# ghnmqdtg/VM-ASR

Measured on AMD Instinct MI355X. Metric: audio clips/sec (train step) 48kHz n_fft=1024, higher is better.
Workload: dtype bf16 (autocast over G; scan/STFT f32; MPD f32/bf16x3 MFMA); 1 GPU; vm_asr_48k_MPD.yaml full train step, DIMS 16 d_state 1 n_fft 1024 clip 122640@48k; per_gpu_batch=4, global_batch=4, parallelism=dp1, execution=hipGraph replay, 2 streams, generator_streams=2

## Files before the change

include/vmasr_hip.h:

```cpp
#ifndef VMASR_HIP_H
#define VMASR_HIP_H

#include <stddef.h>
#include <stdint.h>

#ifdef __cplusplus
extern "C" {
#endif

#define VMASR_ABI_VERSION 1

typedef void *vmasr_stream_t;

enum { VMASR_F32 = 0, VMASR_F16 = 1, VMASR_BF16 = 2 };

enum {
    VMASR_OK = 0,
    VMASR_EINVAL = -1,
    VMASR_EALIGN = -2,
    VMASR_ENOSPACE = -3
};

int vmasr_abi_version(void);
const char *vmasr_last_error(void);
// ... 36 lines not shown
void vmasr_sscan_tune(int rows, int split);

int vmasr_cross_scan(const void *x, void *xs, int32_t B, int32_t C, int32_t H, int32_t W,
                     int32_t dtype, vmasr_stream_t stream);
int vmasr_cross_merge(const void *ys, void *y, int32_t B, int32_t C, int32_t H, int32_t W,
                      int32_t dtype, vmasr_stream_t stream);

int vmasr_cross_scan_cvt(const void *x, void *xs, int32_t B, int32_t C, int32_t H, int32_t W,
                         int32_t in_dtype, int32_t out_dtype, vmasr_stream_t stream);
int vmasr_cross_merge_cvt(const void *ys, void *y, int32_t B, int32_t C, int32_t H, int32_t W,
                          int32_t in_dtype, int32_t out_dtype, vmasr_stream_t stream);

int vmasr_xproj_n_supported(int32_t d_state, int32_t dt_rank, int32_t d_inner);
size_t vmasr_xproj_n_ws_floats(int32_t B, int32_t K, int32_t R, int32_t L);
int vmasr_xproj_n_fwd(const void *xs, const float *Wx, const float *Wdt, float *dts, float *Bs, float *Cs, float *dtr,
                      int32_t B, int32_t K, int32_t D, int32_t N, int32_t R, int32_t L, int32_t dtype, vmasr_stream_t stream);
int vmasr_xproj_n_bwd(const void *xs, const float *Wx, const float *Wdt, const float *dtr, const float *ddts, const float *dBs,
                      const float *dCs, const float *du, void *dxs, float *dWx, float *dWdt, float *ws,
                      int32_t B, int32_t K, int32_t D, int32_t N, int32_t R, int32_t L, int32_t dtype, vmasr_stream_t stream);
int vmasr_xproj_supported(int32_t d_state, int32_t dt_rank, int32_t d_inner);
int vmasr_xproj_fwd(const void *xs, const float *Wx, const float *Wdt, float *dts, float *Bs, float *Cs,
                    float *dtr, int32_t B, int32_t K, int32_t D, int32_t N, int32_t R, int32_t L,
                    int32_t dtype, vmasr_stream_t stream);
int vmasr_xproj_bwd(const void *xs, const float *Wx, const float *Wdt, const float *dtr, const float *ddts,
                    const float *dBs, const float *dCs, const float *du, void *dxs, float *dWx, float *dWdt,
                    float *ws, int32_t B, int32_t K, int32_t D, int32_t N, int32_t R, int32_t L,
                    int32_t dtype, vmasr_stream_t stream);

int vmasr_dwconv_silu_fwd(const void *x, const float *w, const float *bias, void *y, int32_t B,
                          int32_t C, int32_t H, int32_t W, int32_t dtype, vmasr_stream_t stream);
int vmasr_dwconv_silu_bwd(const void *x, const float *w, const float *bias, const void *gy,
                          void *dx, float *dw, float *db, float *ws, int32_t B, int32_t C,
                          int32_t H, int32_t W, int32_t dtype, vmasr_stream_t stream);

int vmasr_stft(const float *wav, float *out0, float *out1, int32_t B, int32_t T, int32_t n_fft,
               int32_t hop, int32_t win, int32_t normalized, int32_t logmag,
               vmasr_stream_t stream);
size_t vmasr_stft_bwd_workspace(int32_t B, int32_t T, int32_t n_fft, int32_t hop);
int vmasr_stft_bwd(const float *gre, const float *gim, float *gwav, int32_t B, int32_t T, int32_t n_fft,
                   int32_t hop, int32_t win, int32_t normalized, void *ws, size_t ws_bytes,
                   vmasr_stream_t stream);
size_t vmasr_istft_workspace(int32_t B, int32_t F, int32_t M, int32_t hop);
int vmasr_istft(const float *mag, const float *phase, float *wav, int32_t B, int32_t F, int32_t M,
                int32_t hop, int32_t win, void *ws, size_t ws_bytes, vmasr_stream_t stream);
int vmasr_istft_bwd(const float *mag, const float *phase, const float *g, float *dmag,
                    float *dphase, int32_t B, int32_t F, int32_t M, int32_t hop, int32_t win,
                    vmasr_stream_t stream);

enum { VMASR_SCALE_LOG2 = 0, VMASR_SCALE_DB = 1 };
size_t vmasr_stft_db_workspace(int32_t B, int32_t T, int32_t n_fft, int32_t hop);
int vmasr_stft_db(const float *wav, float *mag, float *phase, int32_t B, int32_t T, int32_t n_fft, int32_t hop,
                  int32_t win, int32_t normalized, float top_db, void *ws, size_t ws_bytes, vmasr_stream_t stream);
int vmasr_istft_scaled(const float *mag, const float *phase, float *wav, int32_t B, int32_t F, int32_t M, int32_t hop,
                       int32_t win, int32_t scale, void *ws, size_t ws_bytes, vmasr_stream_t stream);
int vmasr_istft_scaled_bwd(const float *mag, const float *phase, const float *g, float *dmag, float *dphase, int32_t B,
                           int32_t F, int32_t M, int32_t hop, int32_t win, int32_t scale, vmasr_stream_t stream);

size_t vmasr_metrics_workspace(int32_t B, int32_t T, int32_t n_fft, int32_t hop);
int vmasr_metrics(const float *out, const float *tgt, const int64_t *hf, float *per_clip, double *acc, int32_t B, int32_t T,
                  int32_t n_fft, int32_t hop, void *ws, size_t ws_bytes, vmasr_stream_t stream);

int vmasr_resample_poly(const float *x, const float *h, float *y, int32_t B, int64_t n_in, int64_t n_out, int32_t up, int32_t down,
                        int32_t half_len, vmasr_stream_t stream);

size_t vmasr_resample_design_workspace(int32_t half_len);
int vmasr_resample_design(float *h, int32_t up, int32_t down, int32_t half_len, void *ws, size_t ws_bytes, vmasr_stream_t stream);
// ... 289 lines not shown

int32_t vmasr_dconv1d_pos_tile(void);
int32_t vmasr_dconv1d_m_tile(void);
int32_t vmasr_dconv1d_k_chunk(void);
int32_t vmasr_dconv1d_max_taps(void);
int vmasr_dconv1d_supported(int32_t Cin, int32_t Cout, int32_t groups, int32_t k, int32_t stride);
int vmasr_dconv1d_supported_launch(int32_t Cin, int32_t Cout, int32_t groups, int32_t k, int32_t stride, int32_t pad, int32_t B, int64_t L);
int32_t vmasr_dconv1d_fwd_slabs(int32_t Cin, int32_t Cout, int32_t groups, int32_t k, int32_t stride, int32_t pad, int32_t B, int64_t L);
size_t vmasr_dconv1d_fwd_workspace(int32_t Cin, int32_t Cout, int32_t groups, int32_t k, int32_t stride, int32_t pad, int32_t B, int64_t L);
size_t vmasr_dconv1d_dgrad_workspace(int32_t Cin, int32_t Cout, int32_t groups, int32_t k, int32_t stride, int32_t pad, int32_t B, int64_t L);
size_t vmasr_dconv1d_wgrad_workspace(int32_t Cin, int32_t Cout, int32_t groups, int32_t k, int32_t stride, int32_t pad, int32_t B, int64_t L);
int vmasr_dconv1d_fwd(const float *x, const float *w, const float *bias, float *y, float *pre, void *ws, size_t ws_bytes, int32_t B,
                      int32_t Cin, int32_t Cout, int32_t groups, int64_t L, int32_t k, int32_t stride, int32_t pad, int32_t act,
                      vmasr_stream_t stream);
int vmasr_dconv1d_dgrad(const float *gy, const float *pre, const float *w, float *dx, void *ws, size_t ws_bytes, int32_t B, int32_t Cin,
                        int32_t Cout, int32_t groups, int64_t L, int32_t k, int32_t stride, int32_t pad, vmasr_stream_t stream);
int vmasr_dconv1d_wgrad(const float *x, const float *gy, const float *pre, float *dw, float *db, void *ws, size_t ws_bytes, int32_t B,
                        int32_t Cin, int32_t Cout, int32_t groups, int64_t L, int32_t k, int32_t stride, int32_t pad, vmasr_stream_t stream);

enum {
    VMASR_K_SSCAN_FWD = 0,
    VMASR_K_SSCAN_FWD_AGG,
    VMASR_K_SSCAN_FWD_CARRY,
    VMASR_K_SSCAN_FWD_APPLY,
    VMASR_K_SSCAN_BWD,
    VMASR_K_SSCAN_BWD_AGG,
    VMASR_K_SSCAN_BWD_CARRY,
    VMASR_K_SSCAN_BWD_APPLY,
    VMASR_K_CROSS_SCAN,
    VMASR_K_CROSS_MERGE,
    VMASR_K_DWCONV_FWD,
    VMASR_K_DWCONV_BWD_A,
    VMASR_K_DWCONV_BWD_B,
    VMASR_K_STFT,
    VMASR_K_ISTFT_FRAMES,
    VMASR_K_ISTFT_OLA,
    VMASR_K_ISTFT_BWD,
    VMASR_K_LN_FWD,
    VMASR_K_LN_BWD,
    VMASR_K_LN_BWD_REDUCE,
    VMASR_K_SMALL_LINEAR_FWD,
    VMASR_K_SMALL_LINEAR_BWD,
    VMASR_K_SMALL_LINEAR_REDUCE,
    VMASR_K_XPROJ_FWD,
    VMASR_K_XPROJ_BWD_A,
    VMASR_K_XPROJ_BWD_B,
    VMASR_K_SPECTRAL,
    VMASR_K_IM2COL,
    VMASR_K_COL2IM,
    VMASR_K_SPLIT_BF16,
    VMASR_K_BIAS_GELU,
    VMASR_K_SS2D_TRANSPOSE,
    VMASR_K_SS2D_FWD_AGG,
    VMASR_K_SS2D_CARRY,
    VMASR_K_SS2D_FWD_APPLY,
    VMASR_K_SS2D_MERGE,
    VMASR_K_SS2D_BWD_AGG,
    VMASR_K_SS2D_BWD_APPLY,
    VMASR_K_SS2D_PRE,
    VMASR_K_LN_GATE,
    VMASR_K_STACK_ROWS,
    VMASR_K_FEAT_L1,
    VMASR_K_ADAMW,
    VMASR_K_CONV_POST,
    VMASR_K_CONV_POST_BWD_GELU,
    VMASR_K_WEIGHT_T,
// ... 59 lines not shown
```

vm_asr_amd/_lib.py:

```python
import ctypes
import os

from . import knobs

_HERE = os.path.dirname(os.path.abspath(__file__))
LIB_PATH = knobs.get("VMASR_LIB") or os.path.join(_HERE, "libvmasr_hip.so")

c_i32, c_i64, c_vp, c_sz = ctypes.c_int32, ctypes.c_int64, ctypes.c_void_p, ctypes.c_size_t

F32, F16, BF16 = 0, 1, 2


class SScanParams(ctypes.Structure):
    _fields_ = (
        [(n, c_i32) for n in ("batch", "dim", "seqlen", "dstate", "n_groups", "n_chunks", "dtype",
                              "delta_softplus")]
        + [(n, c_i64) for n in ("A_d_stride", "A_dstate_stride",
                                "B_batch_stride", "B_group_stride", "B_dstate_stride",
                                "C_batch_stride", "C_group_stride", "C_dstate_stride",
                                "u_batch_stride", "u_d_stride", "delta_batch_stride", "delta_d_stride",
                                "out_batch_stride", "out_d_stride")]
        + [(n, c_vp) for n in ("A_ptr", "B_ptr", "C_ptr", "D_ptr", "u_ptr", "delta_ptr",
                               "delta_bias_ptr", "out_ptr", "x_ptr")]
    )
# ... 135 lines not shown
    "vmasr_ss2d_glue_supported": (ctypes.c_int, [c_i32, c_i32, c_i32]),
    "vmasr_ss2d_pre_fwd": (ctypes.c_int, [c_vp, c_vp, c_vp, c_i32, c_i32, c_i32, c_i32, c_vp]),
    "vmasr_ss2d_pre_bwd": (ctypes.c_int, [c_vp, c_vp, c_vp, c_vp, c_i32, c_i32, c_i32, c_i32, c_vp]),
    "vmasr_ln_gate_fwd": (ctypes.c_int, [c_vp] * 7 + [c_i32, c_i32, c_i32, ctypes.c_float, c_i32, c_vp]),
    "vmasr_ln_gate_bwd": (ctypes.c_int, [c_vp] * 11 + [c_i32, c_i32, c_i32, c_i32, c_vp]),
    "vmasr_ln_gate_bwd_workspace": (c_i64, [c_i32, c_i32, c_i32, c_i32]),
    "vmasr_ln_gate_bwd_ws": (ctypes.c_int, [c_vp] * 12 + [c_i32, c_i32, c_i32, c_i32, c_vp]),
    "vmasr_ln_gate_pair_supported": (ctypes.c_int, [c_i32, c_i32, c_i32]),
    "vmasr_ln_gate_pair_fwd": (ctypes.c_int, [c_vp] * 8 + [c_i32, c_i32, c_i32, c_i32, ctypes.c_float, c_i32, c_vp]),
    "vmasr_ln_gate_pair_bwd": (ctypes.c_int, [c_vp] * 13 + [c_i32, c_i32, c_i32, c_i32, c_i32, c_vp]),
    "vmasr_ss2d_supported": (ctypes.c_int, [c_i32] * 5),
    "vmasr_ss2d_part_floats": (c_sz, [c_i32] * 4),
    "vmasr_ss2d_fwd": (ctypes.c_int, [ctypes.POINTER(SS2DParams), c_vp]),
    "vmasr_ss2d_bwd": (ctypes.c_int, [ctypes.POINTER(SS2DParams), c_vp]),
    "vmasr_ss2d_deep_supported": (ctypes.c_int, [c_i32] * 5),
    "vmasr_ss2d_deep_waves_per_row": (c_i32, [c_i32, c_i32]),
    "vmasr_ss2d_deep_fwd": (ctypes.c_int, [ctypes.POINTER(SS2DDeepParams), c_vp]),
    "vmasr_ss2d_deep_bwd": (ctypes.c_int, [ctypes.POINTER(SS2DDeepParams), c_vp]),
    "vmasr_set_deterministic": (None, [ctypes.c_int]),
    "vmasr_get_deterministic": (ctypes.c_int, []),
    "vmasr_det_timeouts": (ctypes.c_int64, []),
    "vmasr_prof_enable": (None, [ctypes.c_int]),
    "vmasr_prof_reset": (None, []),
    "vmasr_prof_name": (ctypes.c_char_p, [ctypes.c_int]),
    "vmasr_prof_collect": (ctypes.c_int, [ctypes.c_int, ctypes.POINTER(ctypes.c_int64),
                                          ctypes.POINTER(ctypes.c_double), ctypes.POINTER(ctypes.c_double)]),
    "vmasr_prof_collect_shapes": (ctypes.c_int, [ctypes.c_int, ctypes.c_int, ctypes.POINTER(ctypes.c_double), ctypes.POINTER(ctypes.c_int64),
                                                 ctypes.POINTER(ctypes.c_double)]),
    "vmasr_cross_scan": (ctypes.c_int, [c_vp, c_vp, c_i32, c_i32, c_i32, c_i32, c_i32, c_vp]),
    "vmasr_cross_merge": (ctypes.c_int, [c_vp, c_vp, c_i32, c_i32, c_i32, c_i32, c_i32, c_vp]),
    "vmasr_dwconv_silu_fwd": (ctypes.c_int, [c_vp, c_vp, c_vp, c_vp, c_i32, c_i32, c_i32, c_i32, c_i32, c_vp]),
    "vmasr_dwconv_silu_bwd": (ctypes.c_int, [c_vp, c_vp, c_vp, c_vp, c_vp, c_vp, c_vp, c_vp,
                                             c_i32, c_i32, c_i32, c_i32, c_i32, c_vp]),
    "vmasr_stft": (ctypes.c_int, [c_vp, c_vp, c_vp, c_i32, c_i32, c_i32, c_i32, c_i32, c_i32, c_i32, c_vp]),
    "vmasr_stft_bwd_workspace": (c_sz, [c_i32, c_i32, c_i32, c_i32]),
    "vmasr_stft_bwd": (ctypes.c_int, [c_vp, c_vp, c_vp, c_i32, c_i32, c_i32, c_i32, c_i32, c_i32, c_vp, c_sz, c_vp]),
    "vmasr_istft_workspace": (c_sz, [c_i32, c_i32, c_i32, c_i32]),
    "vmasr_istft": (ctypes.c_int, [c_vp, c_vp, c_vp, c_i32, c_i32, c_i32, c_i32, c_i32, c_vp, c_sz, c_vp]),
    "vmasr_istft_bwd": (ctypes.c_int, [c_vp, c_vp, c_vp, c_vp, c_vp, c_i32, c_i32, c_i32, c_i32, c_i32, c_vp]),
    "vmasr_stft_db_workspace": (c_sz, [c_i32, c_i32, c_i32, c_i32]),
    "vmasr_stft_db": (ctypes.c_int, [c_vp, c_vp, c_vp, c_i32, c_i32, c_i32, c_i32, c_i32, c_i32, ctypes.c_float, c_vp, c_sz, c_vp]),
    "vmasr_istft_scaled": (ctypes.c_int, [c_vp, c_vp, c_vp, c_i32, c_i32, c_i32, c_i32, c_i32, c_i32, c_vp, c_sz, c_vp]),
    "vmasr_istft_scaled_bwd": (ctypes.c_int, [c_vp, c_vp, c_vp, c_vp, c_vp, c_i32, c_i32, c_i32, c_i32, c_i32, c_i32, c_vp]),
    "vmasr_metrics_workspace": (c_sz, [c_i32, c_i32, c_i32, c_i32]),
    "vmasr_metrics": (ctypes.c_int, [c_vp, c_vp, c_vp, c_vp, c_vp, c_i32, c_i32, c_i32, c_i32, c_vp, c_sz, c_vp]),
    "vmasr_gconv1d_supported": (ctypes.c_int, [c_i32] * 5),
    "vmasr_gconv1d_supported_launch": (ctypes.c_int, [c_i32] * 7 + [c_i64]),
    "vmasr_gconv1d_wgrad_workspace": (c_sz, [c_i32] * 7 + [c_i64]),
    "vmasr_gconv1d_fwd": (ctypes.c_int, [c_vp] * 5 + [c_i32] * 4 + [c_i64] + [c_i32] * 4 + [c_vp]),
    "vmasr_gconv1d_dgrad": (ctypes.c_int, [c_vp] * 4 + [c_i32] * 4 + [c_i64] + [c_i32] * 3 + [c_vp]),
    "vmasr_gconv1d_wgrad": (ctypes.c_int, [c_vp] * 6 + [c_sz] + [c_i32] * 4 + [c_i64] + [c_i32] * 3 + [c_vp]),
    "vmasr_dconv1d_pos_tile": (c_i32, []),
    "vmasr_dconv1d_m_tile": (c_i32, []),
    "vmasr_dconv1d_k_chunk": (c_i32, []),
    "vmasr_dconv1d_max_taps": (c_i32, []),
    "vmasr_dconv1d_supported": (ctypes.c_int, [c_i32] * 5),
    "vmasr_dconv1d_supported_launch": (ctypes.c_int, [c_i32] * 7 + [c_i64]),
    "vmasr_dconv1d_fwd_slabs": (c_i32, [c_i32] * 7 + [c_i64]),
    "vmasr_dconv1d_fwd_workspace": (c_sz, [c_i32] * 7 + [c_i64]),
    "vmasr_dconv1d_dgrad_workspace": (c_sz, [c_i32] * 7 + [c_i64]),
    "vmasr_dconv1d_wgrad_workspace": (c_sz, [c_i32] * 7 + [c_i64]),
    "vmasr_dconv1d_fwd": (ctypes.c_int, [c_vp] * 6 + [c_sz] + [c_i32] * 4 + [c_i64] + [c_i32] * 4 + [c_vp]),
    "vmasr_dconv1d_dgrad": (ctypes.c_int, [c_vp] * 5 + [c_sz] + [c_i32] * 4 + [c_i64] + [c_i32] * 3 + [c_vp]),
    "vmasr_dconv1d_wgrad": (ctypes.c_int, [c_vp] * 6 + [c_sz] + [c_i32] * 4 + [c_i64] + [c_i32] * 3 + [c_vp]),
    "vmasr_stem1d_time_tile": (c_i32, []),
    "vmasr_stem1d_channel_group": (c_i32, []),
# ... 2 lines not shown
    "vmasr_stem1d_bwd_workspace": (c_sz, [c_i32] * 5 + [c_i64]),
    "vmasr_stem1d_fwd": (ctypes.c_int, [c_vp] * 4 + [c_i32] * 2 + [c_i64] + [c_i32] * 4 + [c_vp]),
    "vmasr_stem1d_bwd": (ctypes.c_int, [c_vp] * 8 + [c_sz] + [c_i32] * 2 + [c_i64] + [c_i32] * 4 + [c_vp]),
    "vmasr_stem1d_fm_supported_launch": (ctypes.c_int, [c_i32] * 5 + [c_i64]),
    "vmasr_stem1d_fm_workspace": (c_sz, [c_i32] * 5 + [c_i64]),
    "vmasr_stem1d_fm_fwd": (ctypes.c_int, [c_vp] * 6 + [c_sz] + [c_i32] * 2 + [c_i64] + [c_i32] * 3 + [c_vp]),
    "vmasr_stem1d_fm_bwd": (ctypes.c_int, [c_vp] * 6 + [ctypes.c_float] + [c_vp] + [c_i32] * 2 + [c_i64] + [c_i32] * 3 + [c_vp]),
    "vmasr_resample_poly": (ctypes.c_int, [c_vp, c_vp, c_vp, c_i32, c_i64, c_i64, c_i32, c_i32, c_i32, c_vp]),
    "vmasr_resample_design_workspace": (c_sz, [c_i32]),
    "vmasr_resample_design": (ctypes.c_int, [c_vp, c_i32, c_i32, c_i32, c_vp, c_sz, c_vp]),
    "vmasr_degrade_batch_workspace": (c_sz, [c_vp, c_i32]),
    "vmasr_degrade_batch": (ctypes.c_int, [c_vp, c_vp, c_vp, c_vp, c_i32, c_i64, c_vp, c_sz, c_vp]),
}

_lib = None


def lib():
    global _lib
    if _lib is None:
        if not os.path.exists(LIB_PATH):
            raise RuntimeError(
                f"{LIB_PATH} is missing: build it with `make -C vm_asr_amd/csrc` "
                "(or __graft_entry__.build()). vm_asr_amd has no CPU fallback.")
        import torch
        l = ctypes.CDLL(LIB_PATH)
        for name, (res, args) in SYMBOLS.items():
            fn = getattr(l, name)
            fn.restype, fn.argtypes = res, args
        if l.vmasr_abi_version() != 1:
            raise RuntimeError("libvmasr_hip.so ABI version mismatch")
        if knobs.get("VMASR_DETERMINISTIC"):
            l.vmasr_set_deterministic(1)
        knobs.warn_undeclared()
        _lib = l
    return _lib


def check(code, what):
    if code != 0:
        msg = lib().vmasr_last_error().decode() or "unknown error"
        raise RuntimeError(f"{what} failed ({code}): {msg}")


def torch_dtype_code(dt):
    import torch
    try:
        return {torch.float32: F32, torch.float16: F16, torch.bfloat16: BF16}[dt]
    except KeyError:
        raise RuntimeError(f"unsupported dtype {dt}: expected float32 / float16 / bfloat16")


def det_mode():
    if knobs.get("VMASR_DETERMINISTIC"):
        return True
    try:
        return bool(lib().vmasr_get_deterministic())
    except (OSError, RuntimeError, AttributeError):
        return False


def current_stream(device):
    import torch
    return ctypes.c_void_p(torch.cuda.current_stream(device).cuda_stream)


# ... 17 lines not shown
            conv[i] = ctypes.c_void_p(a.data_ptr())
        elif isinstance(a, ctypes.Structure):
            conv[i] = ctypes.byref(a)
    if device is None:
        raise RuntimeError(f"{what}: no tensor argument and no device= to launch on")
    with torch.cuda.device(device):
        check(fn(*conv, current_stream(device)), what)


def require_cuda(name, *tensors):
    if not all(t.is_cuda for t in tensors):
        raise RuntimeError(f"{name}: expected a CUDA (HIP) tensor; vm_asr_amd has no CPU path")


def bf16_autocast():
    import torch
    return torch.is_autocast_enabled("cuda") and torch.get_autocast_dtype("cuda") == torch.bfloat16


def autocast_dtype(x):
    import torch
    return torch.get_autocast_dtype("cuda") if torch.is_autocast_enabled("cuda") else x.dtype


def f32c(t, shape):
    return t.detach().float().reshape(shape).contiguous()


def rows2d(t, width):
    t2 = t.reshape(-1, width)
    return t2 if t2.is_contiguous() else t2.contiguous()


K_COUNT = 80


def zeros_f32(device, *shapes):
    import torch
    sizes = [0 if sh is None else -(-int(torch.Size(sh).numel()) // 4) * 4 for sh in shapes]
    flat = torch.zeros(max(1, sum(sizes)), dtype=torch.float32, device=device)
    out, off = [], 0
    for sh, n in zip(shapes, sizes):
        out.append(None if sh is None else flat[off:off + torch.Size(sh).numel()].view(sh))
        off += n
    return out


def prof_enable(on=True):
    lib().vmasr_prof_enable(int(bool(on)))


def prof_reset():
    lib().vmasr_prof_reset()


def prof_collect():
    l = lib()
    out = {}
    for k in range(K_COUNT):
        n, ms, by = ctypes.c_int64(0), ctypes.c_double(0.0), ctypes.c_double(0.0)
        check(l.vmasr_prof_collect(k, ctypes.byref(n), ctypes.byref(ms), ctypes.byref(by)), "prof_collect")
        if n.value:
            out[l.vmasr_prof_name(k).decode()] = dict(launches=n.value, ms=ms.value, alg_bytes=by.value)
    return out


def prof_collect_shapes(name, max_groups=16):
# ... 10 lines not shown
```

vm_asr_amd/csrc/api.hip:

```cpp
#include "common.h"

#include <mutex>
#include <vector>

namespace vmasr {
namespace {
thread_local char g_err[512] = "";

struct Rec {
    int kid;
    hipEvent_t e0, e1;
    double bytes;
};
std::mutex g_mu;
std::vector<Rec> g_recs;
std::vector<hipEvent_t> g_pool;
thread_local Rec g_open{-1, nullptr, nullptr, 0.0};

hipEvent_t take_event() {
    if (!g_pool.empty()) {
        hipEvent_t e = g_pool.back();
        g_pool.pop_back();
        return e;
    }
    hipEvent_t e = nullptr;
    (void)hipEventCreate(&e);
    return e;
}

const char *kNames[VMASR_K_COUNT] = {
    "sscan_fwd", "sscan_fwd_agg", "sscan_fwd_carry", "sscan_fwd_apply", "sscan_bwd", "sscan_bwd_agg",
    "sscan_bwd_carry", "sscan_bwd_apply", "cross_scan", "cross_merge", "dwconv_silu_fwd", "dwconv_silu_bwd_a",
    "dwconv_silu_bwd_b", "stft", "istft_frames", "istft_ola", "istft_bwd", "layer_norm_fwd", "layer_norm_bwd",
    "layer_norm_bwd_reduce", "small_linear_fwd", "small_linear_bwd", "small_linear_reduce",
    "xproj_fwd", "xproj_bwd_a", "xproj_bwd_b", "spectral_power_iter", "im2col_kx1", "col2im_kx1", "split_bf16", "bias_gelu",
    "ss2d_transpose", "ss2d_fwd_agg", "ss2d_carry", "ss2d_fwd_apply", "ss2d_merge", "ss2d_bwd_agg", "ss2d_bwd_apply",
    "ss2d_pre", "ln_gate", "stack_rows", "feat_l1", "adamw", "conv_post", "conv_post_bwd_gelu", "weight_transpose", "mlp_fwd", "mlp_bwd", "gmlp_fwd", "gmlp_bwd", "inproj_fwd", "inproj_bwd",
    "ss2d_deep_xproj", "ss2d_deep_fwd", "ss2d_deep_bwd", "ss2d_deep_xbwd", "outproj_fwd", "outproj_bwd", "stft_loss",
    "conv_mfma_fwd", "conv_mfma_dgrad", "conv_mfma_wgrad", "wgrad_finish", "skinny_linear", "metrics", "resample_design", "degrade_batch",
    "gconv1d_fwd", "gconv1d_dgrad", "gconv1d_wgrad", "gconv1d_wgrad_reduce",
    "stem1d_fwd", "stem1d_bwd", "stem1d_bwd_reduce",
    "dconv1d_fwd", "dconv1d_dgrad", "dconv1d_reduce", "dconv1d_wgrad", "dconv1d_wgrad_reduce", "resample_poly"};
}

bool g_prof_on = false;
static bool g_det_on = false;
constexpr int kMaxDev = 16;
static unsigned *g_det_buf[kMaxDev] = {};

unsigned *det_ticket(int kid) {
    if (!g_det_on || kid < 0 || kid >= VMASR_K_COUNT) return nullptr;
    int dev = 0;
    if (hipGetDevice(&dev) != hipSuccess || dev < 0 || dev >= kMaxDev || g_det_buf[dev] == nullptr) {
        set_error("deterministic mode: no ticket buffer for device %d (vmasr_set_deterministic(1) must run before the first launch)", dev);
        return nullptr;
    }
    return g_det_buf[dev] + kid;
}
static int det_prepare() {
    int n = 0, cur = 0;
    if (hipGetDeviceCount(&n) != hipSuccess || n <= 0) return 0;
    (void)hipGetDevice(&cur);
    int rc = 0;
    for (int d = 0; d < n && d < kMaxDev; ++d) {
        if (g_det_buf[d]) continue;
        if (hipSetDevice(d) != hipSuccess || hipMalloc(reinterpret_cast<void **>(&g_det_buf[d]), 2 * VMASR_K_COUNT * sizeof(unsigned)) != hipSuccess ||
// ... 127 lines not shown
```

vm_asr_amd/csrc/dwconv.hip:

```cpp
#include <algorithm>

#include "common.h"

namespace vmasr {
namespace {

#ifndef VMASR_DW_CHUNK
#define VMASR_DW_CHUNK 2048
#endif
constexpr int kChunk = VMASR_DW_CHUNK;

__device__ __forceinline__ float sigmoid_f(float v) { return __builtin_amdgcn_rcpf(1.f + __expf(-v)); }

template <typename T>
__device__ __forceinline__ float conv_at(const T *__restrict__ xp, const float (&wr)[9], float bias, int h,
                                         int w, int H, int W, float (&taps)[9]) {
    float acc = bias;
#pragma unroll
    for (int i = 0; i < 3; ++i)
#pragma unroll
        for (int j = 0; j < 3; ++j) {
            const int hh = h + i - 1, ww = w + j - 1;
            const float v = (hh >= 0 && hh < H && ww >= 0 && ww < W) ? to_f32(xp[(size_t)hh * W + ww]) : 0.f;
            taps[i * 3 + j] = v;
// ... 175 lines not shown
    }
}

template <typename T>
__global__ __launch_bounds__(256) void dwconv_silu_bwd_b_vec_kernel(const float *__restrict__ gp, const float *__restrict__ w,
                                                                    T *__restrict__ dx, const int C, const int H,
                                                                    const int W, const int chunk) {
    const int c = blockIdx.y, b = blockIdx.z;
    const int HW = H * W;
    const size_t plane = ((size_t)b * C + c) * HW;
    const float *gpp = gp + plane;
    float wr[9];
#pragma unroll
    for (int k = 0; k < 9; ++k) wr[k] = w[c * 9 + k];
    const int l_end = min(HW, (int)(blockIdx.x + 1) * chunk);
    for (int l = blockIdx.x * chunk + threadIdx.x * 4; l < l_end; l += 1024) {
        const int h = l / W, w0 = l - h * W;
        float r0[6], r1[6], r2[6];
        load_row6(gpp + (size_t)(h + 1) * W, h + 1 < H, w0, W, r0);
        load_row6(gpp + (size_t)h * W, true, w0, W, r1);
        load_row6(gpp + (size_t)(h - 1) * W, h > 0, w0, W, r2);
        float o[4];
#pragma unroll
        for (int i = 0; i < 4; ++i) {
            float a = 0.f;
            a = fmaf(wr[0], r0[i + 2], a); a = fmaf(wr[1], r0[i + 1], a); a = fmaf(wr[2], r0[i], a);
            a = fmaf(wr[3], r1[i + 2], a); a = fmaf(wr[4], r1[i + 1], a); a = fmaf(wr[5], r1[i], a);
            a = fmaf(wr[6], r2[i + 2], a); a = fmaf(wr[7], r2[i + 1], a); a = fmaf(wr[8], r2[i], a);
            o[i] = a;
        }
        store4<T, true>(dx + plane, l, HW, o);
    }
}

int check_shape(int B, int C, int H, int W, int dtype, const char *what) {
    VMASR_REQUIRE(B > 0 && C > 0 && H > 0 && W > 0, VMASR_EINVAL, "%s: non-positive size", what);
    VMASR_REQUIRE(B <= 65535 && C <= 65535, VMASR_EINVAL, "%s: B and C must be <= 65535", what);
    VMASR_REQUIRE((long)H * W < (1L << 31), VMASR_EINVAL, "%s: plane too large", what);
    VMASR_REQUIRE(dtype == VMASR_F32 || dtype == VMASR_F16 || dtype == VMASR_BF16, VMASR_EINVAL,
                  "%s: dtype must be fp32/fp16/bf16", what);
    return 0;
}

}
}

using namespace vmasr;

VMASR_EXPORT int vmasr_dwconv_silu_fwd(const void *x, const float *w, const float *bias, void *y, int32_t B,
                                       int32_t C, int32_t H, int32_t W, int32_t dtype, vmasr_stream_t stream) {
    if (int e = check_shape(B, C, H, W, dtype, "dwconv_silu_fwd")) return e;
    VMASR_REQUIRE(x && w && y, VMASR_EINVAL, "dwconv_silu_fwd: null tensor");
    const int chunk = kChunk;
    const dim3 grid((H * W + chunk - 1) / chunk, C, B);
    hipStream_t st = static_cast<hipStream_t>(stream);
    const double bytes = 2.0 * B * C * H * W * (dtype == VMASR_F32 ? 4 : 2);
    const size_t al = dtype == VMASR_F32 ? 16 : 8;
    const bool vec = W % 4 == 0 && aligned_to(x, al) && aligned_to(y, al);
#define VMASR_DW_FWD(TT)                                                                                             \
    do {                                                                                                             \
        if (vec) VMASR_LAUNCH(VMASR_K_DWCONV_FWD, bytes, (dwconv_silu_vec_kernel<TT, 0>), grid, dim3(256), 0, st,     \
                              (const TT *)x, w, bias, (const TT *)nullptr, (TT *)y, (float *)nullptr, (float *)nullptr, \
                              (float *)nullptr, C, H, W, chunk, (unsigned *)nullptr);                                                     \
        else VMASR_LAUNCH(VMASR_K_DWCONV_FWD, bytes, dwconv_silu_fwd_kernel<TT>, grid, dim3(256), 0, st, (const TT *)x, w, \
                          bias, (TT *)y, C, H, W, chunk);                                                            \
    } while (0)
    switch (dtype) {
        case VMASR_F32: VMASR_DW_FWD(float); break;
        case VMASR_F16: VMASR_DW_FWD(f16_t); break;
        default: VMASR_DW_FWD(bf16_t);
    }
#undef VMASR_DW_FWD
    return check_launch("dwconv_silu_fwd");
}

VMASR_EXPORT int vmasr_dwconv_silu_bwd(const void *x, const float *w, const float *bias, const void *gy, void *dx,
                                       float *dw, float *db, float *ws, int32_t B, int32_t C, int32_t H, int32_t W,
                                       int32_t dtype, vmasr_stream_t stream) {
    if (int e = check_shape(B, C, H, W, dtype, "dwconv_silu_bwd")) return e;
    VMASR_REQUIRE(x && w && gy && dx && dw && ws, VMASR_EINVAL, "dwconv_silu_bwd: null tensor");
    const int chunk = kChunk, chunk_a = std::max(kChunk, ((H * W / 64 + 1023) / 1024) * 1024);
    const dim3 grid((H * W + chunk - 1) / chunk, C, B), grid_a((H * W + chunk_a - 1) / chunk_a, C, B);
    hipStream_t st = static_cast<hipStream_t>(stream);
    const double n = (double)B * C * H * W, es = dtype == VMASR_F32 ? 4 : 2;
    const double bytes_a = n * (2 * es + 4), bytes_b = n * (4 + es);
    const size_t al = dtype == VMASR_F32 ? 16 : 8;
    const bool vec = W % 4 == 0 && aligned_to(x, al) && aligned_to(gy, al) && aligned_to(dx, al) && aligned_to(ws, 16);
    unsigned *det = det_ticket(VMASR_K_DWCONV_BWD_A);
#define VMASR_DW_BWD(TT)                                                                                              \
    do {                                                                                                              \
        if (vec) {                                                                                                    \
            VMASR_LAUNCH(VMASR_K_DWCONV_BWD_A, bytes_a, (dwconv_silu_vec_kernel<TT, 1>), grid_a, dim3(256), 0, st,      \
                         (const TT *)x, w, bias, (const TT *)gy, (TT *)nullptr, ws, dw, db, C, H, W, chunk_a, det); \
            VMASR_LAUNCH(VMASR_K_DWCONV_BWD_B, bytes_b, dwconv_silu_bwd_b_vec_kernel<TT>, grid, dim3(256), 0, st, ws, w, \
                         (TT *)dx, C, H, W, chunk);                                                                   \
        } else {                                                                                                      \
            VMASR_LAUNCH(VMASR_K_DWCONV_BWD_A, bytes_a, dwconv_silu_bwd_a_kernel<TT>, grid_a, dim3(256), 0, st, (const TT *)x, \
                         w, bias, (const TT *)gy, ws, dw, db, C, H, W, chunk_a, det);                                 \
            VMASR_LAUNCH(VMASR_K_DWCONV_BWD_B, bytes_b, dwconv_silu_bwd_b_kernel<TT>, grid, dim3(256), 0, st, ws, w,    \
                         (TT *)dx, C, H, W, chunk);                                                                   \
        }                                                                                                             \
    } while (0)
    switch (dtype) {
        case VMASR_F32: VMASR_DW_BWD(float); break;
        case VMASR_F16: VMASR_DW_BWD(f16_t); break;
        default: VMASR_DW_BWD(bf16_t);
    }
#undef VMASR_DW_BWD
    return check_launch("dwconv_silu_bwd");
}
```

vm_asr_amd/knobs.py:

```python
import os
import warnings
from collections import namedtuple

Knob = namedtuple("Knob", "name kind default values reader doc parse")


def _bad(k, raw, allowed):
    return ValueError(f"{k.name}={raw!r}: expected {allowed}")


def _flag(k, raw):
    if raw == "1":
        return True
    if raw == "0":
        return False
    raise _bad(k, raw, "0 or 1")


def _choice(k, raw):
    if raw in k.values:
        return raw
    raise _bad(k, raw, "one of " + " | ".join(k.values))


# ... 43 lines not shown
def _k(name, kind, default, doc, values=None, reader="python", parse=None):
    if kind == "flag":
        values, default = _FLAG_VALUES, bool(default)
    return Knob(name, kind, default, values, reader, doc, parse or _PARSE.get(kind))


def _csrc(name, default, doc):
    return Knob(name, "csrc", default, None, "csrc", doc, None)


def _external(name, doc):
    return Knob(name, "external", None, None, "external", doc, None)


KNOBS = {k.name: k for k in (
    _k("VMASR_LIB", "str", None, "path of the HIP library instead of vm_asr_amd/libvmasr_hip.so (A/B and sanitizer builds); read at import"),
    _k("VMASR_DETERMINISTIC", "flag", 0, "ordered fp32 accumulation everywhere; every stream-layout decision then keeps one stream (_lib.det_mode())"),
    _k("VMASR_LINEAR_F64ACC", "choice", "auto", "fp32 Linear with float64 accumulation: 1 always, 0 never, auto only where no gradient is recorded",
       values=("auto", "0", "1")),
    _k("VMASR_SKINNY", "choice", "1", "streaming kernel for Linear layers of many rows and few features: 1 where it beats the GEMM library, 0 off, "
       "all every supported shape", values=("1", "0", "all")),
    _k("VMASR_SPLITK_CHUNK", "int", 2048, "fewest rows of one K-split of a weight-gradient GEMM; read at import"),
    _k("VMASR_XPROJ_MAX_D", "int", 512, "largest d_inner that takes the x_proj row kernels instead of einsums; read at import"),
    _k("VMASR_FUSED_MLP", "flag", 1, "LayerNorm + Mlp + residual of a VSS block as one operator (mlp.py)"),
    _k("VMASR_FUSED_GMLP", "flag", 1, "LayerNorm + gated Mlp (MODEL.VSSM.GMLP) + residual of a VSS block as one operator (gmlp.py)",
       reader="python:gmlp"),
    _k("VMASR_FUSED_INPROJ", "flag", 1, "LayerNorm + in_proj + split + SiLU as one operator (inproj.py)"),
    _k("VMASR_FUSED_OUTPROJ", "flag", 1, "out_proj + DropPath + residual as one operator (outproj.py)"),
    _k("VMASR_SS2D_FUSED", "flag", 1, "the d_state-1 SS2D core (x_proj, dt_proj, four-direction scan, merge) as one operator (ss2d_core.py)"),
    _k("VMASR_SS2D_DEEP", "flag", 1, "the deep stages' SS2D core on the row-parallel kernels (ss2d_deep.py)"),
    _k("VMASR_SS2D_GLUE", "flag", 1, "the pre-scan and gated-LayerNorm glue kernels (ss2d_glue.py)"),
    _k("VMASR_SS2D_PAIRS", "flag", 1, "magnitude and phase blocks of equal shape through one gated-LayerNorm launch (ss2d_glue.py)"),
    _k("VMASR_IM2COL2D", "flag", 1, "the generator's 2-D convolutions through the row-major im2col kernel (model.py)"),
    _k("VMASR_STFT_LOSS", "flag", 1, "the multi-resolution STFT loss kernel (loss.py)"),
    _k("VMASR_LSGAN", "flag", 1, "the least-squares GAN loss kernel (loss.py)"),
    _k("VMASR_MPD_BATCHED", "flag", 1, "all period discriminators layer by layer on stacked operands"),
    _k("VMASR_MPD_GEMM", "choice", "bf16x3", "fp32 discriminator GEMMs as bf16x3 MFMA triples, or fp32 library GEMMs", values=("bf16x3", "fp32")),
    _k("VMASR_MPD_CONV", "choice", None, "ONE variable read at two sites.  conv_kx1 (one discriminator at a time; unset = unfold): gemm = the "
       "im2col-free GEMM form for stride 3 and stride 1, s3 = that form for the stride-3 layers only, unfold or mfma = unfold + GEMM.  "
       "Batched path (unset = mfma): mfma = the implicit-GEMM MFMA kernels for the compute-bound layers, gemm / s3 / unfold = not those",
       values=("mfma", "gemm", "s3", "unfold")),
    _k("VMASR_MPD_CONV_L1", "choice", "f32", "the 32 -> 128 layer: f32 exact-fp32 MFMA implicit GEMM, 1 bf16x3 pairs, 0 library GEMMs",
       values=("f32", "1", "0")),
    _k("VMASR_MPD_SPLIT_MIN", "int", 1 << 18, "smallest K * N of a stacked layer that takes the split (hi, lo) GEMM path"),
    _k("VMASR_MPD_KCAT", "flag", 0, "the split GEMM's three products as one GEMM over a concatenated K"),
    _k("VMASR_MPD_FUSE_GELU_BWD", "flag", 1, "the activation backward inside the input-gradient epilogue"),
    _k("VMASR_SN_STACK", "flag", 1, "spectral normalisation, stack and permutation of a layer's weights in one launch"),
    _k("VMASR_STACK_INPUT", "flag", 1, "a layer reads the previous layer's stacked output directly"),
    _k("VMASR_CONV_POST", "flag", 1, "the 1-channel output convolution straight on the stacked maps"),
    _k("VMASR_CONV_FIRST", "flag", 1, "the 1 -> 32 channel input convolution + GELU straight from the folded signals"),
    _k("VMASR_FEAT_TAP", "flag", 1, "a feature map's gradient (next layer's + feature-matching loss's) formed in one pass"),
    _k("VMASR_FEAT_L1", "flag", 1, "the feature-matching loss on the stacked maps in one kernel"),
    _k("VMASR_MSD_CONV", "choice", "hip", "the MSD's strided grouped 1-D convolutions: hip = the exact-fp32 MFMA kernels (csrc/gconv1d.hip), "
       "torch = F.conv1d (A/B measurements, double backward)", values=("hip", "torch"), reader="python:msd"),
    _k("VMASR_MSD_STEM", "choice", "hip", "the MSD's 1 -> hidden stem convolution + GELU: hip = one fused pass that keeps no pre-activation "
       "(csrc/stem1d.hip), torch = F.conv1d + F.gelu (A/B measurements, double backward)", values=("hip", "torch"), reader="python:msd"),
    _k("VMASR_MSD_FEAT", "choice", "hip", "the MSD's feature-matching loss in the generator's pass: hip = formed on the way (the stem's share inside "
       "the stem kernels, the other maps in the one-pass L1 kernel; msd_featmatch.py), torch = forward_single + the loop of sub, abs, mean",
       values=("hip", "torch"), reader="python:msd"),
    _k("VMASR_MSD_TAIL", "choice", "torch", "the MSD's dense tail (8h -> 8h k 5 + GELU, conv_post): hip = the exact-fp32 MFMA kernels with ordered "
       "split-K sums (csrc/dconv1d.hip: bit-identical run to run, no library algorithm search), torch = F.conv1d + F.gelu (the default: "
       "faster on the 8h -> 8h layer, profiles/msd_tail.md; double backward)", values=("hip", "torch"), reader="python:msd"),
    _k("VMASR_TWO_STREAM", "choice", "1", "the discriminator on a side stream: 1 on, 0 one stream, force also in deterministic mode (test hook)",
       values=("1", "0", "force")),
    _k("VMASR_SHARE_FAKE_PASS", "flag", 1, "one discriminator pass over the fake batch serves both phases of the step"),
    _k("VMASR_GEN_STREAMS", "choice", "auto", "the generator's phase branch on a stream of its own in captured steps: auto where the trainer says so, "
# ... 59 lines not shown
```

Before: 200.3 clips/s.

## Fuse depthwise conv + SiLU backward into one tiled LDS kernel

Adds a fused backward kernel for the depthwise 3x3 conv + SiLU. Each block recomputes pre-activations over a tile with a one-pixel halo, keeps gy*SiLU'(pre) in LDS, and computes dx, dw and db in the same pass. This replaces the two-pass pair that wrote and re-read an fp32 workspace, cutting global memory traffic and one launch. The cost is halo recomputation, extra LDS use and per-tile syncs. The old path stays available through a knob.

```diff
diff --git a/include/vmasr_hip.h b/include/vmasr_hip.h
--- a/include/vmasr_hip.h
+++ b/include/vmasr_hip.h
@@ -92,6 +92,8 @@
 int vmasr_dwconv_silu_bwd(const void *x, const float *w, const float *bias, const void *gy,
                           void *dx, float *dw, float *db, float *ws, int32_t B, int32_t C,
                           int32_t H, int32_t W, int32_t dtype, vmasr_stream_t stream);
+int32_t vmasr_dwconv_bwd_route(int32_t route);
+int32_t vmasr_dwconv_bwd_tile(int32_t H, int32_t W, int32_t *th, int32_t *tw);
 
 int vmasr_stft(const float *wav, float *out0, float *out1, int32_t B, int32_t T, int32_t n_fft,
                int32_t hop, int32_t win, int32_t normalized, int32_t logmag,
@@ -447,6 +449,7 @@
     VMASR_K_DWCONV_FWD,
     VMASR_K_DWCONV_BWD_A,
     VMASR_K_DWCONV_BWD_B,
+    VMASR_K_DWCONV_BWD_FUSED,
     VMASR_K_STFT,
     VMASR_K_ISTFT_FRAMES,
     VMASR_K_ISTFT_OLA,
diff --git a/vm_asr_amd/_lib.py b/vm_asr_amd/_lib.py
--- a/vm_asr_amd/_lib.py
+++ b/vm_asr_amd/_lib.py
@@ -191,6 +191,8 @@
     "vmasr_dwconv_silu_fwd": (ctypes.c_int, [c_vp, c_vp, c_vp, c_vp, c_i32, c_i32, c_i32, c_i32, c_i32, c_vp]),
     "vmasr_dwconv_silu_bwd": (ctypes.c_int, [c_vp, c_vp, c_vp, c_vp, c_vp, c_vp, c_vp, c_vp,
                                              c_i32, c_i32, c_i32, c_i32, c_i32, c_vp]),
+    "vmasr_dwconv_bwd_route": (c_i32, [c_i32]),
+    "vmasr_dwconv_bwd_tile": (c_i32, [c_i32, c_i32, ctypes.POINTER(c_i32), ctypes.POINTER(c_i32)]),
     "vmasr_stft": (ctypes.c_int, [c_vp, c_vp, c_vp, c_i32, c_i32, c_i32, c_i32, c_i32, c_i32, c_i32, c_vp]),
     "vmasr_stft_bwd_workspace": (c_sz, [c_i32, c_i32, c_i32, c_i32]),
     "vmasr_stft_bwd": (ctypes.c_int, [c_vp, c_vp, c_vp, c_i32, c_i32, c_i32, c_i32, c_i32, c_i32, c_vp, c_sz, c_vp]),
@@ -259,6 +261,7 @@
             raise RuntimeError("libvmasr_hip.so ABI version mismatch")
         if knobs.get("VMASR_DETERMINISTIC"):
             l.vmasr_set_deterministic(1)
+        l.vmasr_dwconv_bwd_route(1 if knobs.get("VMASR_DWCONV_BWD") == "split" else 0)
         knobs.warn_undeclared()
         _lib = l
     return _lib
@@ -342,7 +345,7 @@
     return t2 if t2.is_contiguous() else t2.contiguous()
 
 
-K_COUNT = 80
+K_COUNT = 81
 
 
 def zeros_f32(device, *shapes):
diff --git a/vm_asr_amd/csrc/api.hip b/vm_asr_amd/csrc/api.hip
--- a/vm_asr_amd/csrc/api.hip
+++ b/vm_asr_amd/csrc/api.hip
@@ -31,7 +31,7 @@
 const char *kNames[VMASR_K_COUNT] = {
     "sscan_fwd", "sscan_fwd_agg", "sscan_fwd_carry", "sscan_fwd_apply", "sscan_bwd", "sscan_bwd_agg",
     "sscan_bwd_carry", "sscan_bwd_apply", "cross_scan", "cross_merge", "dwconv_silu_fwd", "dwconv_silu_bwd_a",
-    "dwconv_silu_bwd_b", "stft", "istft_frames", "istft_ola", "istft_bwd", "layer_norm_fwd", "layer_norm_bwd",
+    "dwconv_silu_bwd_b", "dwconv_silu_bwd_fused", "stft", "istft_frames", "istft_ola", "istft_bwd", "layer_norm_fwd", "layer_norm_bwd",
     "layer_norm_bwd_reduce", "small_linear_fwd", "small_linear_bwd", "small_linear_reduce",
     "xproj_fwd", "xproj_bwd_a", "xproj_bwd_b", "spectral_power_iter", "im2col_kx1", "col2im_kx1", "split_bf16", "bias_gelu",
     "ss2d_transpose", "ss2d_fwd_agg", "ss2d_carry", "ss2d_fwd_apply", "ss2d_merge", "ss2d_bwd_agg", "ss2d_bwd_apply",
diff --git a/vm_asr_amd/csrc/dwconv.hip b/vm_asr_amd/csrc/dwconv.hip
--- a/vm_asr_amd/csrc/dwconv.hip
+++ b/vm_asr_amd/csrc/dwconv.hip
@@ -231,6 +231,137 @@
         store4<T, true>(dx + plane, l, HW, o);
     }
 }
+
+constexpr int kFusedTile = 4096;
+constexpr int kFusedTW = 512;
+
+struct FusedTiling {
+    int th, tw, ntx, ntiles, nq_max;
+    size_t lds_bytes;
+};
+inline FusedTiling fused_tiling(int H, int W) {
+    FusedTiling t;
+    t.tw = std::min(W, kFusedTW);
+    t.th = std::max(1, std::min(H, kFusedTile / t.tw));
+    t.ntx = (W + t.tw - 1) / t.tw;
+    t.ntiles = t.ntx * ((H + t.th - 1) / t.th);
+    t.nq_max = t.tw / 4 + (t.ntx > 1 ? 2 : 0);
+    t.lds_bytes = (size_t)(t.th + 2) * t.nq_max * 6 * sizeof(float);
+    return t;
+}
+
+__device__ __forceinline__ void lds_row6(const float4 *__restrict__ s_gp, const float *__restrict__ s_first,
+                                         const float *__restrict__ s_last, bool row_ok, int r, int q, int nq, bool has_l,
+                                         bool has_r, float (&v)[6]) {
+    if (!row_ok) {
+#pragma unroll
+        for (int i = 0; i < 6; ++i) v[i] = 0.f;
+        return;
+    }
+    const int k = r * nq + q;
+    const float4 g = s_gp[k];
+    v[0] = has_l ? s_last[k - 1] : 0.f;
+    v[1] = g.x; v[2] = g.y; v[3] = g.z; v[4] = g.w;
+    v[5] = has_r ? s_first[k + 1] : 0.f;
+}
+
+template <typename T>
+__global__ __launch_bounds__(256) void dwconv_silu_bwd_fused_kernel(const T *__restrict__ x, const float *__restrict__ w,
+                                                                    const float *__restrict__ bias, const T *__restrict__ gy,
+                                                                    T *__restrict__ dx, float *__restrict__ dw, float *__restrict__ db,
+                                                                    const int C, const int H, const int W, const int th, const int tw,
+                                                                    const int ntx, const int ntiles, const int nq_max, unsigned *det) {
+    extern __shared__ float4 s_dyn[];
+    __shared__ float s_part[4][10];
+    float4 *s_gp = s_dyn;
+    float *s_first = reinterpret_cast<float *>(s_dyn + (th + 2) * nq_max);
+    float *s_last = s_first + (th + 2) * nq_max;
+    const int c = blockIdx.y, b = blockIdx.z;
+    const int HW = H * W;
+    const size_t plane = ((size_t)b * C + c) * HW;
+    const T *xp = x + plane;
+    float wr[9], acc[10];
+#pragma unroll
+    for (int k = 0; k < 9; ++k) wr[k] = w[c * 9 + k];
+#pragma unroll
+    for (int k = 0; k < 10; ++k) acc[k] = 0.f;
+    const float bv = bias ? bias[c] : 0.f;
+    for (int t = blockIdx.x; t < ntiles; t += gridDim.x) {
+        const int ty = t / ntx, tx = t - ty * ntx;
+        const int h_lo = ty * th, h_hi = min(H, h_lo + th), w_lo = tx * tw, w_hi = min(W, w_lo + tw);
+        const int eh_lo = max(h_lo - 1, 0), eh_hi = min(h_hi + 1, H);
+        const int eq_lo = max(w_lo / 4 - 1, 0), eq_hi = min(w_hi / 4 + 1, W / 4);
+        const int nq = eq_hi - eq_lo, n1 = (eh_hi - eh_lo) * nq;
+        for (int k = threadIdx.x; k < n1; k += 256) {
+            const int r = k / nq, q = k - r * nq;
+            const int h = eh_lo + r, w0 = 4 * (eq_lo + q);
+            float r0[6], r1[6], r2[6], g4[4], o[4];
+            load_row6(xp + (size_t)(h - 1) * W, h > 0, w0, W, r0);
+            load_row6(xp + (size_t)h * W, true, w0, W, r1);
+            load_row6(xp + (size_t)(h + 1) * W, h + 1 < H, w0, W, r2);
+            load4<T, true>(gy + plane, h * W + w0, HW, g4);
+            const bool own = h >= h_lo && h < h_hi && w0 >= w_lo && w0 < w_hi;
+#pragma unroll
+            for (int i = 0; i < 4; ++i) {
+                float pre = bv;
+                pre = fmaf(wr[0], r0[i], pre); pre = fmaf(wr[1], r0[i + 1], pre); pre = fmaf(wr[2], r0[i + 2], pre);
+                pre = fmaf(wr[3], r1[i], pre); pre = fmaf(wr[4], r1[i + 1], pre); pre = fmaf(wr[5], r1[i + 2], pre);
+                pre = fmaf(wr[6], r2[i], pre); pre = fmaf(wr[7], r2[i + 1], pre); pre = fmaf(wr[8], r2[i + 2], pre);
+                const float sg = sigmoid_f(pre);
+                const float g = g4[i] * (sg * (1.f + pre * (1.f - sg)));
+                o[i] = g;
+                if (own) {
+                    acc[0] = fmaf(g, r0[i], acc[0]); acc[1] = fmaf(g, r0[i + 1], acc[1]); acc[2] = fmaf(g, r0[i + 2], acc[2]);
+                    acc[3] = fmaf(g, r1[i], acc[3]); acc[4] = fmaf(g, r1[i + 1], acc[4]); acc[5] = fmaf(g, r1[i + 2], acc[5]);
+                    acc[6] = fmaf(g, r2[i], acc[6]); acc[7] = fmaf(g, r2[i + 1], acc[7]); acc[8] = fmaf(g, r2[i + 2], acc[8]);
+                    acc[9] += g;
+                }
+            }
+            s_gp[k] = make_float4(o[0], o[1], o[2], o[3]);
+            s_first[k] = o[0];
+            s_last[k] = o[3];
+        }
+        __syncthreads();
+        const int tq = (w_hi - w_lo) / 4, n2 = (h_hi - h_lo) * tq;
+        const int r_off = h_lo - eh_lo, q_off = w_lo / 4 - eq_lo;
+        for (int k = threadIdx.x; k < n2; k += 256) {
+            const int rr = k / tq, qq = k - rr * tq;
+            const int h = h_lo + rr, w0 = w_lo + 4 * qq;
+            const int r = r_off + rr, q = q_off + qq;
+            const bool has_l = w0 > 0, has_r = w0 + 4 < W;
+            float r0[6], r1[6], r2[6], o[4];
+            lds_row6(s_gp, s_first, s_last, h + 1 < H, r + 1, q, nq, has_l, has_r, r0);
+            lds_row6(s_gp, s_first, s_last, true, r, q, nq, has_l, has_r, r1);
+            lds_row6(s_gp, s_first, s_last, h > 0, r - 1, q, nq, has_l, has_r, r2);
+#pragma unroll
+            for (int i = 0; i < 4; ++i) {
+                float a = 0.f;
+                a = fmaf(wr[0], r0[i + 2], a); a = fmaf(wr[1], r0[i + 1], a); a = fmaf(wr[2], r0[i], a);
+                a = fmaf(wr[3], r1[i + 2], a); a = fmaf(wr[4], r1[i + 1], a); a = fmaf(wr[5], r1[i], a);
+                a = fmaf(wr[6], r2[i + 2], a); a = fmaf(wr[7], r2[i + 1], a); a = fmaf(wr[8], r2[i], a);
+                o[i] = a;
+            }
+            store4<T, true>(dx + plane, h * W + w0, HW, o);
+        }
+        if (t + (int)gridDim.x < ntiles) __syncthreads();
+    }
+    const int lane = threadIdx.x & 63, wave = threadIdx.x >> 6;
+#pragma unroll
+    for (int k = 0; k < 10; ++k) {
+        const float sres = wave_sum(acc[k]);
+        if (lane == 0) s_part[wave][k] = sres;
+    }
+    __syncthreads();
+    det_enter(det);
+    if (threadIdx.x < 10) {
+        const float sres = s_part[0][threadIdx.x] + s_part[1][threadIdx.x] + s_part[2][threadIdx.x] + s_part[3][threadIdx.x];
+        if (threadIdx.x < 9) atomicAdd(dw + c * 9 + threadIdx.x, sres);
+        else if (db) atomicAdd(db + c, sres);
+    }
+    det_leave(det);
+}
+
+int g_bwd_route = 0;
 
 int check_shape(int B, int C, int H, int W, int dtype, const char *what) {
     VMASR_REQUIRE(B > 0 && C > 0 && H > 0 && W > 0, VMASR_EINVAL, "%s: non-positive size", what);
@@ -286,9 +417,16 @@
     const size_t al = dtype == VMASR_F32 ? 16 : 8;
     const bool vec = W % 4 == 0 && aligned_to(x, al) && aligned_to(gy, al) && aligned_to(dx, al) && aligned_to(ws, 16);
     unsigned *det = det_ticket(VMASR_K_DWCONV_BWD_A);
+    const bool fused = vec && g_bwd_route == 0;
+    const FusedTiling ft = fused_tiling(H, W);
+    const dim3 grid_f(std::min(ft.ntiles, (int)grid_a.x), C, B);
 #define VMASR_DW_BWD(TT)                                                                                              \
     do {                                                                                                              \
-        if (vec) {                                                                                                    \
+        if (fused) {                                                                                                  \
+            VMASR_LAUNCH(VMASR_K_DWCONV_BWD_FUSED, n * 3 * es, dwconv_silu_bwd_fused_kernel<TT>, grid_f, dim3(256),    \
+                         ft.lds_bytes, st, (const TT *)x, w, bias, (const TT *)gy, (TT *)dx, dw, db, C, H, W, ft.th, ft.tw, \
+                         ft.ntx, ft.ntiles, ft.nq_max, det);                                                          \
+        } else if (vec) {                                                                                             \
             VMASR_LAUNCH(VMASR_K_DWCONV_BWD_A, bytes_a, (dwconv_silu_vec_kernel<TT, 1>), grid_a, dim3(256), 0, st,      \
                          (const TT *)x, w, bias, (const TT *)gy, (TT *)nullptr, ws, dw, db, C, H, W, chunk_a, det); \
             VMASR_LAUNCH(VMASR_K_DWCONV_BWD_B, bytes_b, dwconv_silu_bwd_b_vec_kernel<TT>, grid, dim3(256), 0, st, ws, w, \
@@ -308,3 +446,16 @@
 #undef VMASR_DW_BWD
     return check_launch("dwconv_silu_bwd");
 }
+
+VMASR_EXPORT int32_t vmasr_dwconv_bwd_route(int32_t route) {
+    if (route == 0 || route == 1) g_bwd_route = route;
+    return g_bwd_route;
+}
+
+VMASR_EXPORT int32_t vmasr_dwconv_bwd_tile(int32_t H, int32_t W, int32_t *th, int32_t *tw) {
+    if (H <= 0 || W <= 0 || W % 4 != 0 || (long)H * W >= (1L << 31)) return 0;
+    const FusedTiling ft = fused_tiling(H, W);
+    if (th) *th = ft.th;
+    if (tw) *tw = ft.tw;
+    return ft.ntiles;
+}
diff --git a/vm_asr_amd/knobs.py b/vm_asr_amd/knobs.py
--- a/vm_asr_amd/knobs.py
+++ b/vm_asr_amd/knobs.py
@@ -99,6 +99,9 @@
     _k("VMASR_SS2D_GLUE", "flag", 1, "the pre-scan and gated-LayerNorm glue kernels (ss2d_glue.py)"),
     _k("VMASR_SS2D_PAIRS", "flag", 1, "magnitude and phase blocks of equal shape through one gated-LayerNorm launch (ss2d_glue.py)"),
     _k("VMASR_IM2COL2D", "flag", 1, "the generator's 2-D convolutions through the row-major im2col kernel (model.py)"),
+    _k("VMASR_DWCONV_BWD", "choice", "fused", "the depthwise conv + SiLU backward: fused = one kernel that keeps gy * SiLU'(pre) in LDS wherever "
+       "the vectorised case holds (csrc/dwconv.hip), split = always the two-pass pair through the fp32 workspace (A/B measurements); handed to "
+       "the library once, when it is loaded (vmasr_dwconv_bwd_route switches it later)", values=("fused", "split"), reader="python:dwconv"),
     _k("VMASR_STFT_LOSS", "flag", 1, "the multi-resolution STFT loss kernel (loss.py)"),
     _k("VMASR_LSGAN", "flag", 1, "the least-squares GAN loss kernel (loss.py)"),
     _k("VMASR_MPD_BATCHED", "flag", 1, "all period discriminators layer by layer on stacked operands"),
```

Result: no change. 201.0 clips/s, median of 6 (+0.3%).
